# SIA-IDE/MMGT

Measured on AMD Instinct MI355X. Metric: UNet3D denoise-steps/sec at 512x512x24 bf16, higher is better.
Workload: dtype bf16; 1 GPU; BASELINE configs[1]: 512x512x24 pose2vid denoise step (CFG batch 2, UNet3D + MM-HAA, 16 reference banks, 1 window of 24 frames, guidance 3.5, DDIM v-pred), random-init weights; frames=24, parallelism=clip-parallel x1

## Files before the change

include/mmgt_hip.h:

```cpp
#ifndef MMGT_HIP_H
#define MMGT_HIP_H

#ifdef __cplusplus
extern "C" {
#endif

#define MMGT_F32 0
#define MMGT_BF16 1

#define MMGT_ACT_NONE 0
#define MMGT_ACT_GEGLU 1
#define MMGT_ACT_SILU 2
#define MMGT_ACT_RELU 3
#define MMGT_ACT_QUICK_GELU 4
#define MMGT_ACT_GELU 5
#define MMGT_ACT_MISH 6

int mmgt_abi_version(void);
const char* mmgt_last_error(void);
int mmgt_tune(const char* key, int value);
int mmgt_tune_get(const char* key, int* value);
int mmgt_box_calib(float warm_seconds, float* mfma_mhz, float* mfma_tflops, void* stream);
void mmgt_gemm16_set_trace(void* p);
void mmgt_ffn_set_trace(void* p);
// ... 84 lines not shown
                       int F, int hw, float guidance, float sa_t, float sb_t, float sa_p, float sb_p, void* stream);

int mmgt_accumulate_window(const void* pred, float* pred_sum, float* counter, const int* idx, int Fw, int F, int C,
                           int Cpad, int hw, int dtype, void* stream);

int mmgt_accumulate_window_rows(const void* pred, float* pred_sum, float* counter, const int* idx, int Fw, int F, int C,
                                int Cpad, int hw, int rows, int row0, int bump_counter, int dtype, void* stream);

int mmgt_accumulate_windows(const void* pred, float* pred_sum, float* counter, const int* idx, int B, int Fw, int F, int C, int Cpad,
                            int hw, int dtype, void* stream);

int mmgt_rotary(const void* x, const float* cos_sin, void* out, long rows, int dim, int seq, int dtype, void* stream);
int mmgt_film_residual(const void* x, const float* scale_shift, long ld_ss, const void* res, const void* res2, void* out, long rows,
                       int dim, int rows_per_batch, int dtype, void* stream);
int mmgt_mean_tokens(const void* x, float* out, int batch, int tokens, int dim, int dtype, void* stream);
int mmgt_activation(const void* x, void* out, long n, int act, int dtype, void* stream);
int mmgt_smga_ddim_step(const void* pred_uncond, const void* pred_cond, const float* x, const float* noise, float* out, long n,
                        float guidance, float sqrt_recip_acp, float sqrt_recipm1_acp, float sqrt_acp_next, float c, float sigma,
                        int last, int dtype, void* stream);

long mmgt_temporal_leg320_image_bytes(void);
int mmgt_temporal_leg320(const void* x, void* out, const float* ln_gamma, const float* beta_pe, int pe_rows, const void* wimg, const float* bias_o,
                         int batch, int frames, int n_pix, float scale, float eps, int dtype, void* stream);

long mmgt_gn_silu_conv3x3_image_bytes(int cin, int cout);
int mmgt_gn_silu_conv3x3(const void* x, const float* scale, const float* shift, const void* wimg, const float* bias, const void* residual, void* out,
                         float* stats, int nb, int H, int W, int cin, int cout, int ldo, int dtype, void* stream);
int mmgt_gn_stats_finalize(const float* stats, const float* gamma, const float* beta, float* scale, float* shift, int nb, int tiles, int C, int G,
                           float eps, void* stream);

long mmgt_gn_silu_conv3x3_unet_image_bytes(int cin, int cout);
int mmgt_gn_silu_conv3x3_unet_stats_rows(int nb, int H, int W, int cout);
int mmgt_gn_silu_conv3x3_unet_stats(const void* x0, int C0, const void* x1, int C1, const float* scale_shift, const void* wimg, const float* bias,
                                    const float* bias2, int b2_imgs, const void* residual, void* out, float* stats, int nb, int H, int W, int cout, int dtype,
                                    void* stream);
int mmgt_gn_stats_finalize_unet(const float* stats, const float* gamma, const float* beta, float* scale_shift, int nb, int parts_per_img, int count, int C,
                                int G, float eps, void* stream);
void mmgt_rconv_set_trace(void* buf);
int mmgt_gn_silu_conv3x3_unet(const void* x0, int C0, const void* x1, int C1, const float* scale_shift, const void* wimg, const float* bias,
                              const float* bias2, int b2_imgs, const void* residual, void* out, int nb, int H, int W, int cout, int dtype, void* stream);

int mmgt_blur_mask_u8(const unsigned char* masks, unsigned char* out, int frames, int H, int W, int ksize, void* stream);
int mmgt_resample_u8(const unsigned char* in, float* out_f32, unsigned char* out_u8, int frames, int S, int D, const int* bounds,
                     const int* coeffs, int ksize, void* stream);
int mmgt_window_stack(const float* x, float* out, int frames, long D, int half, void* stream);
int mmgt_frames_to_u8(const void* x, unsigned char* out, long npix, int cpad, float scale, float shift, int dtype, void* stream);
// ... 59 lines not shown
```

mmgt_amd/csrc/gemm.hip:

```cpp
#include <string.h>

#include <type_traits>

#include "common.h"
#include "gemm_common.h"
#include "mmgt_hip.h"

#ifndef MMGT_GEMM_VARIANT
#define MMGT_GEMM_VARIANT 7
#endif

namespace {

constexpr bool V_FRAGDB = (MMGT_GEMM_VARIANT & 1) != 0;
constexpr bool V_ILV = (MMGT_GEMM_VARIANT & 2) != 0;
constexpr bool V_LATE = (MMGT_GEMM_VARIANT & 4) != 0;
constexpr bool V_LATE_ALL = (MMGT_GEMM_VARIANT & 8) != 0;
constexpr bool V_NODMA = (MMGT_GEMM_VARIANT & 16) != 0;

template <int CTRL>
__device__ __forceinline__ unsigned dpp_quad(unsigned v) {
  return (unsigned)__builtin_amdgcn_mov_dpp((int)v, CTRL, 0xf, 0xf, true);
}
template <int S>
// ... 738 lines not shown
  MMGT_CHECK(M > 0 && N > 0 && K > 0, "gemm: empty problem M=%d N=%d K=%d", M, N, K);
  MMGT_CHECK(K % 64 == 0, "gemm: K=%d must be a multiple of 64 (pad channels on the host)", K);
  MMGT_CHECK(act >= 0 && act <= 6, "gemm: bad act %d", act);
  MMGT_CHECK(act != 1 || N % 64 == 0, "gemm: GEGLU needs N %% 64 == 0 (N=%d)", N);
  return 0;
}

}

void mmgt_attn_set64(int v);
void mmgt_gn_set_rows(int v);
void mmgt_attn_set_heads_inner(int v);
void mmgt_attn_set_attn80(int v);
void mmgt_attn_set_nomax(int v);
void mmgt_gemm16_set_pb(int v);
void mmgt_gemm16_set_stagger(int v);
void mmgt_gn_set_interleave(int v);
void mmgt_gn_set_lpr0(int v);
void mmgt_gn_set_narrow(int v);
void mmgt_gn_set_slab(int v);
void mmgt_ffn_set_dbg(int v);
void mmgt_rowgemm_set_dbg(int v);
void mmgt_tleg_set_abl(int v);
void mmgt_gnconv_set_abl(int v);
void mmgt_rconv_set_abl(int v);
void mmgt_rconv_set_stagger(int v);
void mmgt_rconv_set_cb(int v);
namespace {
struct HostSwitch { const char* key; int value; };
HostSwitch g_host[] = {
    {"fused_ff", 1},
    {"twin_attention", 1},
    {"shared_rows", 1},
    {"oz3", 1},
    {"rowgemm", 1},
    {"tleg", 1},
    {"rconv", 5},
    {"conv_out_taps", 1},
    {"ffpo_cat", 1},
    {"sc_cat", 1},
    {"up2", 1},
    {"rconv_stats", 1},
    {"gnconv", 2},
    {"zero_audio_skip", 1},
    {"window_state", 1},
    {"smga_graph", 1},
};
}
extern "C" int mmgt_tune_get(const char* key, int* value) {
  if (key && value)
    for (const HostSwitch& h : g_host)
      if (!strcmp(key, h.key)) { *value = h.value; return 0; }
  mmgt_set_error("tune_get: unknown key");
  return 1;
}
extern "C" int mmgt_tune(const char* key, int value) {
  if (key)
    for (HostSwitch& h : g_host)
      if (!strcmp(key, h.key)) { h.value = value; return 0; }
  if (key && !strcmp(key, "gemm_cfg")) { g_gemm_cfg = value; return 0; }
  if (key && !strcmp(key, "attn64")) { mmgt_attn_set64(value); return 0; }
  if (key && !strcmp(key, "attn_nomax") && (value == 0 || value == 1)) { mmgt_attn_set_nomax(value); return 0; }
  if (key && !strcmp(key, "attn_heads_inner")) { mmgt_attn_set_heads_inner(value); return 0; }
  if (key && !strcmp(key, "attn80")) { mmgt_attn_set_attn80(value); return 0; }
  if (key && !strcmp(key, "g16_pb")) { mmgt_gemm16_set_pb(value); return 0; }
  if (key && !strcmp(key, "g16_stagger")) { mmgt_gemm16_set_stagger(value); return 0; }
  if (key && !strcmp(key, "gn_rows")) { mmgt_gn_set_rows(value); return 0; }
  if (key && !strcmp(key, "gn_interleave")) { mmgt_gn_set_interleave(value); return 0; }
  if (key && !strcmp(key, "gn_narrow")) { mmgt_gn_set_narrow(value); return 0; }
  if (key && !strcmp(key, "gn_slab")) { mmgt_gn_set_slab(value); return 0; }
  if (key && !strcmp(key, "gn_lpr0")) { if (value != 4 && value != 8 && value != 16) return -1; mmgt_gn_set_lpr0(value); return 0; }
  if (key && !strcmp(key, "splitk")) { g_splitk = value; return 0; }
  if (key && !strcmp(key, "bm192")) { g_bm192 = value; return 0; }
  if (key && !strcmp(key, "tailsplit")) { g_tailsplit = value; return 0; }
  if (key && !strcmp(key, "rconv_cb") && (value == 0 || value == 320 || value == 256 || value == 160)) { mmgt_rconv_set_cb(value); return 0; }
  if (key && !strcmp(key, "rconv_stagger") && value >= 0 && value <= 8192) { mmgt_rconv_set_stagger(value); return 0; }
#ifdef MMGT_ABLATE
  if (key && !strcmp(key, "ffn_dbg") && value >= 0 && value <= 2) { mmgt_ffn_set_dbg(value); return 0; }
  if (key && !strcmp(key, "gnconv_abl") && value >= 0 && value <= 255) { mmgt_gnconv_set_abl(value); return 0; }
  if (key && !strcmp(key, "tleg_abl") && value >= 0 && value <= 128) { mmgt_tleg_set_abl(value); return 0; }
  if (key && !strcmp(key, "rconv_abl") && value >= 0 && value <= 31) { mmgt_rconv_set_abl(value); return 0; }
  if (key && !strcmp(key, "rowgemm_dbg") && value >= 0 && value <= 5) { mmgt_rowgemm_set_dbg(value); return 0; }
#else
  if (key && !strcmp(key, "rowgemm_dbg") && (value == 0 || value == 5)) { mmgt_rowgemm_set_dbg(value); return 0; }
  if (key && (!strcmp(key, "ffn_dbg") || !strcmp(key, "gnconv_abl") || !strcmp(key, "tleg_abl") || !strcmp(key, "rconv_abl") || !strcmp(key, "rowgemm_dbg"))) {
    mmgt_set_error("tune: '%s' selects a timing ablation whose results are garbage; the product library does not contain them (build libmmgt_hip_abl.so with `make -C mmgt_amd/csrc abl` and load it through MMGT_LIB)", key);
    return 1;
  }
#endif
// ... 156 lines not shown
```

mmgt_amd/hip.py:

```python
import ctypes
import os
from ctypes import c_float, c_int, c_long, c_void_p

import torch

_HERE = os.path.dirname(os.path.abspath(__file__))
LIB_PATH = os.environ.get("MMGT_LIB") or os.path.join(_HERE, "libmmgt_hip.so")

F32, BF16 = 0, 1
ACT_NONE, ACT_GEGLU, ACT_SILU, ACT_RELU, ACT_QUICK_GELU, ACT_GELU, ACT_MISH = 0, 1, 2, 3, 4, 5, 6

_lib = None
DMA_LIMIT = (1 << 31) - 1

_SIGS = {
    "mmgt_abi_version": (c_int, []),
    "mmgt_last_error": (ctypes.c_char_p, []),
    "mmgt_tune": (c_int, [ctypes.c_char_p, c_int]),
    "mmgt_tune_get": (c_int, [ctypes.c_char_p, ctypes.POINTER(c_int)]),
    "mmgt_box_calib": (c_int, [c_float, ctypes.POINTER(c_float), ctypes.POINTER(c_float), c_void_p]),
    "mmgt_gemm16_set_trace": (None, [c_void_p]),
    "mmgt_ffn_set_trace": (None, [c_void_p]),
    "mmgt_rconv_set_trace": (None, [c_void_p]),
    "mmgt_gemm": (c_int, [c_void_p, c_long, c_void_p, c_void_p, c_void_p, c_int, c_void_p, c_float, c_void_p, c_long,
# ... 32 lines not shown
    "mmgt_ff_fused": (c_int, [c_void_p, c_long, c_void_p, c_void_p, c_float, c_void_p, c_void_p, c_void_p, c_long, c_void_p, c_long,
                              c_int, c_int, c_int, c_int, c_void_p]),
    "mmgt_rowgemm320_image_bytes": (c_long, [c_int]),
    "mmgt_rowgemm_set_trace": (None, [c_void_p]),
    "mmgt_ff_fused_po": (c_int, [c_void_p, c_long, c_void_p, c_void_p, c_float, c_void_p, c_void_p, c_void_p, c_long, c_void_p, c_void_p,
                                 c_void_p, c_long, c_void_p, c_long, c_int, c_int, c_int, c_int, c_void_p]),
    "mmgt_groupnorm_affine": (c_int, [c_void_p, c_int, c_void_p, c_void_p, c_void_p, c_void_p, c_void_p, c_int, c_int, c_int, c_float, c_int,
                                      c_void_p]),
    "mmgt_rowgemm320": (c_int, [c_void_p, c_long, c_int, c_void_p, c_void_p, c_int, c_int, c_float, c_void_p, c_void_p, c_void_p, c_int, c_void_p,
                                c_long, c_void_p, c_long, c_int, c_void_p, c_int, c_int, c_int, c_int, c_int, c_void_p]),
    "mmgt_gn_silu_conv3x3_image_bytes": (c_long, [c_int, c_int]),
    "mmgt_gn_silu_conv3x3": (c_int, [c_void_p, c_void_p, c_void_p, c_void_p, c_void_p, c_void_p, c_void_p, c_void_p, c_int, c_int, c_int, c_int, c_int, c_int, c_int, c_void_p]),
    "mmgt_gn_silu_conv3x3_unet_image_bytes": (c_long, [c_int, c_int]),
    "mmgt_gn_silu_conv3x3_unet": (c_int, [c_void_p, c_int, c_void_p, c_int, c_void_p, c_void_p, c_void_p, c_void_p, c_int, c_void_p, c_void_p,
                                          c_int, c_int, c_int, c_int, c_int, c_void_p]),
    "mmgt_gn_silu_conv3x3_unet_stats_rows": (c_int, [c_int, c_int, c_int, c_int]),
    "mmgt_gn_silu_conv3x3_unet_stats": (c_int, [c_void_p, c_int, c_void_p, c_int, c_void_p, c_void_p, c_void_p, c_void_p, c_int, c_void_p, c_void_p, c_void_p,
                                                c_int, c_int, c_int, c_int, c_int, c_void_p]),
    "mmgt_gn_stats_finalize_unet": (c_int, [c_void_p, c_void_p, c_void_p, c_void_p, c_int, c_int, c_int, c_int, c_int, c_float, c_void_p]),
    "mmgt_groupnorm_affine2": (c_int, [c_void_p, c_int, c_void_p, c_int, c_void_p, c_void_p, c_void_p, c_void_p, c_void_p, c_int, c_int, c_int,
                                       c_float, c_int, c_void_p]),
    "mmgt_gn_stats_finalize": (c_int, [c_void_p, c_void_p, c_void_p, c_void_p, c_void_p, c_int, c_int, c_int, c_int, c_float, c_void_p]),
    "mmgt_temporal_leg320_image_bytes": (c_long, []),
    "mmgt_temporal_leg320": (c_int, [c_void_p, c_void_p, c_void_p, c_void_p, c_int, c_void_p, c_void_p, c_int, c_int, c_int, c_float, c_float, c_int,
                                     c_void_p]),
    "mmgt_channel_norm_gelu": (c_int, [c_void_p, c_void_p, c_void_p, c_void_p, c_int, c_int, c_float, c_int, c_void_p]),
    "mmgt_lerp_rows": (c_int, [c_void_p, c_void_p, c_int, c_int, c_int, c_int, c_void_p]),
    "mmgt_relpos_attention": (c_int, [c_void_p, c_long, c_long, c_void_p, c_long, c_long, c_void_p, c_long, c_long, c_void_p, c_long, c_long,
                                      c_void_p, c_long, c_long, c_void_p, c_void_p, c_void_p, c_void_p, c_int, c_int, c_int, c_int, c_float,
                                      c_int, c_void_p]),
    "mmgt_silu": (c_int, [c_void_p, c_void_p, c_long, c_int, c_void_p]),
    "mmgt_cfg_ddim_step": (c_int, [c_void_p, c_void_p, c_void_p, c_void_p, c_long, c_int, c_int, c_float, c_float,
                                   c_float, c_float, c_float, c_void_p]),
    "mmgt_accumulate_window": (c_int, [c_void_p, c_void_p, c_void_p, c_void_p, c_int, c_int, c_int, c_int, c_int, c_int,
                                       c_void_p]),
    "mmgt_rotary": (c_int, [c_void_p, c_void_p, c_void_p, c_long, c_int, c_int, c_int, c_void_p]),
    "mmgt_film_residual": (c_int, [c_void_p, c_void_p, c_long, c_void_p, c_void_p, c_void_p, c_long, c_int, c_int, c_int, c_void_p]),
    "mmgt_mean_tokens": (c_int, [c_void_p, c_void_p, c_int, c_int, c_int, c_int, c_void_p]),
    "mmgt_activation": (c_int, [c_void_p, c_void_p, c_long, c_int, c_int, c_void_p]),
    "mmgt_smga_ddim_step": (c_int, [c_void_p, c_void_p, c_void_p, c_void_p, c_void_p, c_long, c_float, c_float, c_float, c_float,
                                    c_float, c_float, c_int, c_int, c_void_p]),
    "mmgt_blur_mask_u8": (c_int, [c_void_p, c_void_p, c_int, c_int, c_int, c_int, c_void_p]),
    "mmgt_resample_u8": (c_int, [c_void_p, c_void_p, c_void_p, c_int, c_int, c_int, c_void_p, c_void_p, c_int, c_void_p]),
    "mmgt_window_stack": (c_int, [c_void_p, c_void_p, c_int, c_long, c_int, c_void_p]),
    "mmgt_frames_to_u8": (c_int, [c_void_p, c_void_p, c_long, c_int, c_float, c_float, c_int, c_void_p]),
    "mmgt_jpeg_dct_quant": (c_int, [c_void_p, c_void_p, c_int, c_int, c_int, c_int, c_int, c_void_p]),
# ... 498 lines not shown

def temporal_leg320_supported(dtype, C, heads, frames, n_pix, batch=1):
    return dtype == torch.bfloat16 and C == 320 and heads == 8 and frames in (12, 24) and n_pix % (4 * 48 // frames) == 0 and \
        batch * frames * n_pix * 640 < (1 << 31)


def temporal_leg320(x, ln_gamma, beta_pe, wimg, bias_o, batch, frames, n_pix, scale, eps=1e-5, out=None):
    _dev(x, ln_gamma, beta_pe, wimg, bias_o, out)
    if not (x.dim() == 2 and temporal_leg320_supported(x.dtype, x.shape[1], 8, frames, n_pix, batch)):
        raise RuntimeError(f"temporal_leg320: unsupported shape (dtype {x.dtype}, {tuple(x.shape)}, {frames} frames x {n_pix} pixels x batch {batch}): "
                           "8 heads of 40 channels, 12 or 24 frames, bf16, < 2 GiB")
    assert x.dim() == 2 and x.shape == (batch * frames * n_pix, 320) and x.is_contiguous() and x.dtype == torch.bfloat16
    assert wimg.dtype == torch.uint8 and wimg.is_contiguous() and wimg.numel() == lib().mmgt_temporal_leg320_image_bytes()
    assert beta_pe.dim() == 2 and beta_pe.shape[1] == 320 and beta_pe.shape[0] >= frames
    if out is None:
        out = torch.empty_like(x)
    assert out.shape == x.shape and out.is_contiguous() and out.dtype == x.dtype
    _check(lib().mmgt_temporal_leg320(_ptr(x), _ptr(out), _ptr(_f32(ln_gamma, "ln_gamma")), _ptr(_f32(beta_pe, "beta_pe")), beta_pe.shape[0],
                                      _ptr(wimg), _ptr(_f32(bias_o, "bias_o")), batch, frames, n_pix, scale, eps, dtype_code(x.dtype), _stream()),
           "mmgt_temporal_leg320")
    return out



def attention(q, k, v, out, *, batch, heads, hd, nq, nk, scale, q_str, k_str, v_str, o_str, bdiv=1, v_transposed=False,
              k2=None, v2=None, k2_str=(0, 0), v2_str=(0, 0), k2_bdiv=1, nk2=0, seg2_first_batch=0, out_scale=None, out_scale_heads=0,
              twin_out=None):
    _dev(q, k, v, out, k2, v2, out_scale, twin_out)
    if twin_out is not None:
        assert k2 is not None and v_transposed and seg2_first_batch == 0 and out_scale is None and twin_out.dtype == out.dtype
        _check(lib().mmgt_attention_twin(_ptr(q), q_str[0], q_str[1], q_str[2], _ptr(k), k_str[0], k_str[1], k_str[2], _ptr(v),
                                         v_str[0], v_str[1], v_str[2], _ptr(out), _ptr(twin_out), o_str[0], o_str[1], o_str[2], bdiv,
                                         _ptr(k2), _ptr(v2), k2_str[0], k2_str[1], v2_str[0], v2_str[1], k2_bdiv, nk2, batch, heads, hd,
                                         nq, nk, scale, dtype_code(q.dtype), _stream()), "mmgt_attention_twin")
        return out
    if out_scale is not None:
        assert k2 is None and not v_transposed and bdiv == 1 and out_scale_heads > 0 and heads % out_scale_heads == 0
        assert out_scale.dtype == torch.float32 and out_scale.dim() == 2 and out_scale.stride(1) == 1
        assert out_scale.shape == (heads // out_scale_heads, batch * nq)
        _check(lib().mmgt_attention_scaled(_ptr(q), q_str[0], q_str[1], q_str[2], _ptr(k), k_str[0], k_str[1], k_str[2], _ptr(v),
                                           v_str[0], v_str[1], v_str[2], _ptr(out), o_str[0], o_str[1], o_str[2], _ptr(out_scale),
                                           out_scale.stride(0), out_scale_heads, batch, heads, hd, nq, nk, scale, dtype_code(q.dtype),
                                           _stream()), "mmgt_attention_scaled")
        return out
    _check(lib().mmgt_attention(_ptr(q), q_str[0], q_str[1], q_str[2], _ptr(k), k_str[0], k_str[1], k_str[2], _ptr(v),
                                v_str[0], v_str[1], v_str[2], _ptr(out), o_str[0], o_str[1], o_str[2], bdiv, _ptr(k2),
# ... 836 lines not shown
```

mmgt_amd/packing.py:

```python
import torch


def pack_geglu(w, b):
    n2, k = w.shape
    n = n2 // 2
    assert n % 32 == 0
    wp = w.reshape(2, n // 32, 32, k).permute(1, 0, 2, 3).reshape(n2, k).contiguous()
    bp = None if b is None else b.reshape(2, n // 32, 32).permute(1, 0, 2).reshape(n2).contiguous()
    return wp, bp


def pack_conv3x3(w, cin_pad=None, cout_pad=None):
    cout, cin = w.shape[:2]
    cin_pad = cin_pad or cin
    cout_pad = cout_pad or cout
    out = torch.zeros((cout_pad, 3, 3, cin_pad), device=w.device, dtype=w.dtype)
    out[:cout, :, :, :cin] = w.permute(0, 2, 3, 1)
    return out.contiguous()


def pack_conv3x3_up2(w):
    cout, cin = w.shape[:2]
    wf = w if w.dtype == torch.float64 else w.float()
    groups = (((0,), (1, 2)), ((0, 1), (2,)))
# ... 117 lines not shown
        for w in bf:
            chunks.append(frags(w, wide))
            chunks.append(torch.zeros(2048, device=dev, dtype=torch.uint8))
        for w in bf:
            chunks.append(frags(w, narrow))
    ch = torch.empty((C // 32, 64, 8), device=dev, dtype=torch.long)
    jj, lqq = j[None, :], lq[:, None]
    for k in range(H):
        ch[k] = HD * k + torch.where(jj < 4, 4 * lqq + jj, 16 + 4 * lqq + jj - 4)
    for u in range(2):
        head = 4 * u + torch.where(jj < 4, 0, 2) + (lqq >= 2).long()
        ch[8 + u] = HD * head + 32 + 4 * (lqq & 1) + (jj & 3)
    wob = wo.to(torch.bfloat16)
    nt = torch.arange(2, device=dev)
    for oc in range(C // 32):
        rows = 32 * oc + 16 * nt[:, None] + lm[None, :]
        img = wob[rows[None, :, :, None], ch[:, None, :, :]]
        chunks.append(img.contiguous().view(torch.uint8).reshape(-1))
    out = torch.cat(chunks)
    assert out.numel() == 4 * (3 * 32768 + 3 * 20480) + 10 * 20480
    return out


def pack_gnconv(w):
    cout, cin = w.shape[0], w.shape[1]
    assert tuple(w.shape) == (cout, cin, 3, 3) and (cin, cout) in ((128, 128), (256, 128), (256, 256), (128, 64))
    dev = w.device
    cl = min(cout, 128)
    lane = torch.arange(64, device=dev)
    rows = 16 * torch.arange(cl // 16, device=dev)[:, None] + (lane & 15)[None, :]
    kk = torch.arange(4, device=dev)
    cols = 32 * kk[:, None, None] + 8 * (lane >> 4)[None, :, None] + torch.arange(8, device=dev)[None, None, :]
    wt = w.to(torch.bfloat16).permute(2, 3, 0, 1).reshape(9, cout, cin)
    img = torch.stack([torch.stack([wt[:, cl * blk + rows[None, :, :, None], 128 * ph + cols[:, None, :, :]] for ph in range(cin // 128)])
                       for blk in range(cout // cl)])
    return img.contiguous().view(torch.uint8).reshape(-1)


def pack_rconv(w):
    cout, cin = w.shape[0], w.shape[1]
    assert tuple(w.shape) == (cout, cin, 3, 3) and cin % 64 == 0 and cout % 16 == 0
    wt = w.to(torch.bfloat16).permute(2, 3, 0, 1).reshape(9, cout // 16, 16, cin // 64, 2, 4, 8)
    img = wt.permute(3, 0, 4, 1, 5, 2, 6)
    return img.contiguous().view(torch.uint8).reshape(-1)
```

mmgt_amd/unet3d.py:

```python
import math
from dataclasses import dataclass
from typing import Dict, List, Optional, Union

import torch

from . import hip
from .packing import pack_conv3x3, pack_conv3x3_up2, pack_conv_taps, pack_ff_fused, pack_ff_proj_out, pack_geglu, pack_rconv, pack_rowgemm, pack_tleg, pad_cols, pad_rows, round_up
from .unet3d_spec import unet3d_spec

SD15_CONFIG = dict(
    in_channels=4, out_channels=4, block_out_channels=(320, 640, 1280, 1280), layers_per_block=2, attention_head_dim=8,
    cross_attention_dim=768, audio_attention_dim=768, norm_num_groups=32, norm_eps=1e-5, center_input_sample=False,
    use_motion_module=True, use_audio_module=True, use_inflated_groupnorm=True,
    motion_module_kwargs=dict(num_attention_heads=8, temporal_position_encoding_max_len=32),
)


@dataclass
class UNet3DConditionOutput:
    sample: torch.Tensor

    def __getitem__(self, i):
        return (self.sample,)[i]


RCONV_LEVEL = {320: 1, 640: 2, 1280: 4}


class _Config(dict):
    __getattr__ = dict.__getitem__
# ... 62 lines not shown
        self.config = _Config(cfg)
        boc = tuple(cfg["block_out_channels"])
        if len(boc) != 4 or any(c % 64 for c in boc) or any((c // 8) not in (40, 80, 160) for c in boc):
            raise ValueError(f"block_out_channels {boc}: the HIP kernels cover head dims 40/80/160 (SD-1.5 widths)")
        self.boc = boc
        self.heads = 8
        self.in_channels = cfg["in_channels"]
        self.out_channels = cfg["out_channels"]
        self._device = torch.device(device)
        self._dtype = dtype
        hip.dtype_code(dtype)
        self.training = True
        self.gradient_checkpointing = False
        self._fuse_ff = bool(hip.tune_get("fused_ff"))
        self._twin = bool(hip.tune_get("twin_attention"))
        self._share_rows = bool(hip.tune_get("shared_rows"))
        self._fuse_oz = bool(hip.tune_get("oz3"))
        self._fuse_ln = bool(hip.tune_get("rowgemm"))
        self._ffpo_cat = bool(hip.tune_get("ffpo_cat"))
        self._ffpo = {}
        self._sc_cat = bool(hip.tune_get("sc_cat"))
        self._up2 = bool(hip.tune_get("up2"))
        self._fuse_tleg = bool(hip.tune_get("tleg"))
        self._rconv_stats = bool(hip.tune_get("rconv_stats"))
        self._rconv = hip.tune_get("rconv")
        self.spec = unet3d_spec(boc, cfg["cross_attention_dim"], cfg["audio_attention_dim"], self.in_channels,
                                self.out_channels, cfg["layers_per_block"],
                                cfg["motion_module_kwargs"].get("temporal_position_encoding_max_len", 32))
        self.w: Dict[str, torch.Tensor] = {}
        self._banks: Dict[str, tuple] = {}
        self.bank_fp16_roundtrip = dtype == torch.float32
        self._loaded = False
        self._ehs_cache = None
        self._zbias = {}

    @classmethod
    def from_config(cls, config, **kwargs):
        config = dict(config)
        config.update(kwargs)
        dev = config.pop("device", "cuda")
        dt = config.pop("dtype", torch.bfloat16)
        return cls(device=dev, dtype=dt, **config)

    @classmethod
    def from_pretrained_2d(cls, pretrained_model_path, motion_module_path, subfolder=None, unet_additional_kwargs=None,
                           mm_zero_proj_out=False, device="cuda", dtype=torch.bfloat16):
# ... 236 lines not shown
                w[t + ".oz3.wb"] = self._t(pad).contiguous()
            ff(t + ".ff")

        self._motion = [k[: -len(".temporal_transformer.norm.weight")] for k in self.spec
                        if k.endswith(".temporal_transformer.norm.weight")]
        for p in self._motion:
            q = p + ".temporal_transformer"
            t = q + ".transformer_blocks.0"
            norm(q + ".norm")
            lin(q + ".proj_in")
            proj_in_img(q)
            lin(q + ".proj_out")
            for i in range(2):
                a = f"{t}.attention_blocks.{i}"
                if has(a + ".to_q.weight"):
                    w[a + ".qkv.w"] = self._t(torch.cat([sd[a + ".to_q.weight"], sd[a + ".to_k.weight"],
                                                         sd[a + ".to_v.weight"]], 0))
                    rowimg(a + ".qkv_img", [sd[a + ".to_q.weight"], sd[a + ".to_k.weight"], sd[a + ".to_v.weight"]])
                    if self._fuse_tleg and has(a + ".to_out.0.weight") and has(a + ".to_out.0.bias") and \
                            hip.temporal_leg320_supported(self._dtype, sd[a + ".to_q.weight"].shape[1], self.heads, 24, 4096):
                        w[a + ".tleg_img"] = pack_tleg(*(sd[a + k].to(self._device) for k in (".to_q.weight", ".to_k.weight", ".to_v.weight",
                                                                                               ".to_out.0.weight")))
                lin(a + ".to_out.0", a + ".o")
                if has(a + ".pos_encoder.pe"):
                    w[a + ".pe"] = self._f(sd[a + ".pos_encoder.pe"][0])
                norm(f"{t}.norms.{i}")
                if (a + ".pe") in w and (f"{t}.norms.{i}.b") in w:
                    w[f"{t}.norms.{i}.bpe"] = (w[f"{t}.norms.{i}.b"][None, :] + w[a + ".pe"]).contiguous()
            norm(t + ".ff_norm")
            ff(t + ".ff")

    def bank_keys(self) -> List[str]:
        down = [p for p in self._spatial if p.startswith("down_blocks")]
        up = [p for p in self._spatial if p.startswith("up_blocks")]
        mid = [p for p in self._spatial if p.startswith("mid_block")]
        return down + up + mid

    def set_banks(self, banks: Optional[Dict[str, torch.Tensor]]):
        self._banks = {}
        if not banks:
            return
        for p, bank in banks.items():
            if p not in self._spatial:
                raise KeyError(f"set_banks: {p} is not a reference-attention reader")
            t = p + ".transformer_blocks.0.attn1"
            bk = bank.to(self._device)
# ... 340 lines not shown
    def _motion_module(self, p, x, frames):
        nb, h, ww, c = x.shape
        n = h * ww
        m = nb * n
        b = nb // frames
        hd = c // self.heads
        if frames > 32:
            raise RuntimeError("temporal attention window is limited to 32 frames (positional encoding max_len)")
        q = p + ".temporal_transformer"
        t = q + ".transformer_blocks.0"
        hid = self._norm_proj_in(q, x)
        for i in range(2):
            a = f"{t}.attention_blocks.{i}"
            if (a + ".tleg_img") in self.w and (f"{t}.norms.{i}.bpe") in self.w and hip.temporal_leg320_supported(self._dtype, c, self.heads, frames, n, b):
                hid = hip.temporal_leg320(hid, self.w[f"{t}.norms.{i}.g"], self.w[f"{t}.norms.{i}.bpe"], self.w[a + ".tleg_img"], self.w[a + ".o.bias"],
                                          b, frames, n, hd ** -0.5)
                continue
            if (a + ".qkv_img") in self.w and n % 128 == 0:
                qkv, _ = hip.rowgemm320(hid, self.w[a + ".qkv_img"], 3 * c, ln_gamma=self.w[f"{t}.norms.{i}.g"],
                                        ln_beta=self.w[f"{t}.norms.{i}.bpe"], pe_div=n, pe_mod=frames)
            else:
                nrm = hip.layernorm(hid, self.w[f"{t}.norms.{i}.g"], self.w[f"{t}.norms.{i}.bpe"], 1e-5, pe_div=n, pe_mod=frames)
                qkv = hip.gemm(nrm, self.w[a + ".qkv.w"])
            o = torch.empty((m, c), device=self._device, dtype=self._dtype)
            st = (frames * n * 3 * c, 3 * c, n * 3 * c)
            hip.attention(qkv, qkv[:, c:], qkv[:, 2 * c:], o, batch=b * n, heads=self.heads, hd=hd, nq=frames, nk=frames,
                          scale=hd ** -0.5, q_str=st, k_str=st, v_str=st, o_str=(frames * n * c, c, n * c), bdiv=n)
            hid = hip.gemm(o, self.w[a + ".o.w"], self.w[a + ".o.bias"], residual=hid)
        out = self._norm_ff_proj_out(t + ".ff", t + ".ff_norm", hid, q, x.view(m, c))
        return out.view(nb, h, ww, c)

    def _time_embedding(self, timestep, batch):
        if not torch.is_tensor(timestep):
            ts = torch.tensor([float(timestep)], dtype=torch.float32, device=self._device)
        else:
            ts = timestep.to(device=self._device, dtype=torch.float32).reshape(-1)
        if ts.numel() == 1:
            batch = 1
        ts = ts.expand(batch).contiguous()
        feat = hip.timestep_features(ts, self.boc[0], self._dtype)
        e = self._lin("time_embedding.linear_1", feat, act=hip.ACT_SILU)
        e = self._lin("time_embedding.linear_2", e)
        all_t = hip.gemm(hip.silu(e), self.w["temb_all.w"], self.w["temb_all.bias"]).float()
        return {p: all_t[:, off:off + n].contiguous() for p, (off, n) in self._temb_slices.items()}

    def forward(self, sample, timestep, encoder_hidden_states, audio_embedding=None, class_labels=None,
# ... 110 lines not shown
```

Before: 15.04 steps/s.

## Fuse temporal attention, output projection, bias and residual into one kernel

Adds a HIP kernel for temporal self-attention at the 640- and 1280-channel levels. Each block does the per-pixel 24-frame attention for all 8 heads into LDS, then runs the output-projection GEMM from a prepacked weight image, adding bias and the residual. This drops the attention-output round trip to global memory and one GEMM launch per temporal leg. The default switch value enables it only for the 640-channel level; it also adds an optional sleep-based stagger for the first wave of blocks and extra weight memory for the packed images.

```diff
diff --git a/include/mmgt_hip.h b/include/mmgt_hip.h
--- a/include/mmgt_hip.h
+++ b/include/mmgt_hip.h
@@ -130,6 +130,10 @@
 long mmgt_temporal_leg320_image_bytes(void);
 int mmgt_temporal_leg320(const void* x, void* out, const float* ln_gamma, const float* beta_pe, int pe_rows, const void* wimg, const float* bias_o,
                          int batch, int frames, int n_pix, float scale, float eps, int dtype, void* stream);
+
+long mmgt_temporal_tail_image_bytes(int C);
+int mmgt_temporal_tail(const void* qkv, const void* hid, void* out, const void* wimg, const float* bias_o, int batch, int frames, int n_pix,
+                       int C, int heads, float scale, int dtype, void* stream);
 
 long mmgt_gn_silu_conv3x3_image_bytes(int cin, int cout);
 int mmgt_gn_silu_conv3x3(const void* x, const float* scale, const float* shift, const void* wimg, const float* bias, const void* residual, void* out,
diff --git a/mmgt_amd/csrc/gemm.hip b/mmgt_amd/csrc/gemm.hip
--- a/mmgt_amd/csrc/gemm.hip
+++ b/mmgt_amd/csrc/gemm.hip
@@ -784,6 +784,7 @@
 void mmgt_ffn_set_dbg(int v);
 void mmgt_rowgemm_set_dbg(int v);
 void mmgt_tleg_set_abl(int v);
+void mmgt_ttail_set_stagger(int v);
 void mmgt_gnconv_set_abl(int v);
 void mmgt_rconv_set_abl(int v);
 void mmgt_rconv_set_stagger(int v);
@@ -797,6 +798,7 @@
     {"oz3", 1},
     {"rowgemm", 1},
     {"tleg", 1},
+    {"ttail", 1},
     {"rconv", 5},
     {"conv_out_taps", 1},
     {"ffpo_cat", 1},
@@ -827,6 +829,7 @@
   if (key && !strcmp(key, "attn80")) { mmgt_attn_set_attn80(value); return 0; }
   if (key && !strcmp(key, "g16_pb")) { mmgt_gemm16_set_pb(value); return 0; }
   if (key && !strcmp(key, "g16_stagger")) { mmgt_gemm16_set_stagger(value); return 0; }
+  if (key && !strcmp(key, "ttail_stagger") && value >= -1 && value <= 16) { mmgt_ttail_set_stagger(value); return 0; }
   if (key && !strcmp(key, "gn_rows")) { mmgt_gn_set_rows(value); return 0; }
   if (key && !strcmp(key, "gn_interleave")) { mmgt_gn_set_interleave(value); return 0; }
   if (key && !strcmp(key, "gn_narrow")) { mmgt_gn_set_narrow(value); return 0; }
diff --git a/mmgt_amd/csrc/ttail.hip b/mmgt_amd/csrc/ttail.hip
--- /dev/null
+++ b/mmgt_amd/csrc/ttail.hip
@@ -0,0 +1,332 @@
+#include <type_traits>
+
+#include "common.h"
+#include "gemm_common.h"
+#include "mmgt_hip.h"
+
+namespace {
+
+typedef __attribute__((ext_vector_type(4))) float acc4;
+
+constexpr int TT_HEADS = 8, TT_GT = 10, TT_RING = 16;
+
+struct TtailArgs {
+  const bf16_t* qkv;
+  const bf16_t* hid;
+  bf16_t* out;
+  const char* wimg;
+  const float* bias;
+  int n, tasks_per_batch;
+  unsigned qkv_bytes, hid_bytes, img_bytes;
+  float scale_log2e;
+  int stagger, first_round;
+};
+
+__device__ __forceinline__ acc4 tt_mma(s16x8 a, s16x8 b, acc4 c) { return __builtin_amdgcn_mfma_f32_16x16x32_bf16(a, b, c, 0, 0, 0); }
+__device__ __forceinline__ s16x8 tt_frag(u32x4 u) {
+  union { u32x4 u; s16x8 s; } cv;
+  cv.u = u;
+  return cv.s;
+}
+__device__ __forceinline__ s16x8 tt_frag2(u32x2 lo, u32x2 hi) { return tt_frag((u32x4){lo[0], lo[1], hi[0], hi[1]}); }
+__device__ __forceinline__ u32x2 tt_pack4(acc4 v) { return (u32x2){pack_bf16x2(v[0], v[1]), pack_bf16x2(v[2], v[3])}; }
+__device__ __forceinline__ float tt_lo(unsigned u) { return __uint_as_float(u << 16); }
+__device__ __forceinline__ float tt_hi(unsigned u) { return __uint_as_float(u & 0xffff0000u); }
+__device__ __forceinline__ float tt_quad_sum(float v) {
+  const auto a = __builtin_amdgcn_permlane16_swap(__float_as_uint(v), __float_as_uint(v), false, false);
+  v = __uint_as_float(a[0]) + __uint_as_float(a[1]);
+  const auto b = __builtin_amdgcn_permlane32_swap(__float_as_uint(v), __float_as_uint(v), false, false);
+  return __uint_as_float(b[0]) + __uint_as_float(b[1]);
+}
+__device__ __forceinline__ float tt_quad_max(float v) {
+  const auto a = __builtin_amdgcn_permlane16_swap(__float_as_uint(v), __float_as_uint(v), false, false);
+  v = fmaxf(__uint_as_float(a[0]), __uint_as_float(a[1]));
+  const auto b = __builtin_amdgcn_permlane32_swap(__float_as_uint(v), __float_as_uint(v), false, false);
+  return fmaxf(__uint_as_float(b[0]), __uint_as_float(b[1]));
+}
+
+template <int F> constexpr bool tt_pair(int kt, int qt) { return (16 * kt) / F <= (16 * qt + 15) / F && (16 * qt) / F <= (16 * kt + 15) / F; }
+template <int F> constexpr bool tt_all(int kt, int qt) { return (16 * kt) / F == (16 * kt + 15) / F && (16 * qt) / F == (16 * qt + 15) / F && (16 * kt) / F == (16 * qt) / F; }
+
+template <int C> constexpr int tt_rows() { return C == 640 ? 48 : 24; }
+template <int C> constexpr int tt_lds() { return tt_rows<C>() * (C * 2 + 16); }
+
+template <int C, int F>
+__global__ __launch_bounds__(256) __attribute__((amdgpu_waves_per_eu(2, 2)))
+void ttail_kernel(const TtailArgs a) {
+  constexpr int R = tt_rows<C>(), NRT = (R + 15) / 16, P = R / F;
+  constexpr int HD = C / TT_HEADS, KSH = (HD + 31) / 32, NCH = HD / 16;
+  constexpr int RS = C * 2 + 16, NKS = C / 32, NG = C / (4 * 16 * TT_GT);
+  static_assert(R % F == 0 && F % 4 == 0 && HD % 16 == 0 && NKS % 2 == 0 && NG >= 1, "geometry");
+  extern __shared__ __attribute__((aligned(16))) char smem[];
+  const int tid = threadIdx.x, lane = tid & 63, wid = __builtin_amdgcn_readfirstlane(tid >> 6);
+  const int lm = lane & 15, lq = lane >> 4;
+  using std::integral_constant;
+#define TT_IC(v) integral_constant<int, (v)>{}
+  auto for_range = [](auto LOc, auto HIc, auto&& fn) {
+    constexpr int lo = decltype(LOc)::value, hi = decltype(HIc)::value;
+    [&]<int... I>(std::integer_sequence<int, I...>) { (fn(integral_constant<int, lo + I>{}), ...); }(std::make_integer_sequence<int, (hi > lo ? hi - lo : 0)>{});
+  };
+
+  const __amdgpu_buffer_rsrc_t rq = __builtin_amdgcn_make_buffer_rsrc(const_cast<bf16_t*>(a.qkv), 0, (int)a.qkv_bytes, 0x00020000);
+  const __amdgpu_buffer_rsrc_t rh = __builtin_amdgcn_make_buffer_rsrc(const_cast<bf16_t*>(a.hid), 0, (int)a.hid_bytes, 0x00020000);
+  const __amdgpu_buffer_rsrc_t ro = __builtin_amdgcn_make_buffer_rsrc(a.out, 0, (int)a.hid_bytes, 0x00020000);
+  const __amdgpu_buffer_rsrc_t rw = __builtin_amdgcn_make_buffer_rsrc(const_cast<char*>(a.wimg), 0, (int)a.img_bytes, 0x00020000);
+
+  if (a.stagger > 0 && (int)blockIdx.x >= a.first_round / 2 && (int)blockIdx.x < a.first_round) {
+    for (int i = 0; i < a.stagger; ++i) __builtin_amdgcn_s_sleep(127);
+  }
+
+  const int task = blockIdx.x;
+  const int b = task / a.tasks_per_batch, p0 = (task - b * a.tasks_per_batch) * P;
+  unsigned qoff[NRT], hoff[NRT];
+#pragma unroll
+  for (int rt = 0; rt < NRT; ++rt) {
+    const int rho = 16 * rt + lm, rc = rho < R ? rho : R - 1;
+    const int px = rc / F, f = rc - px * F;
+    const unsigned grow = (unsigned)((b * F + f) * a.n + p0 + px);
+    qoff[rt] = grow * (unsigned)(3 * C * 2);
+    hoff[rt] = grow * (unsigned)(C * 2);
+  }
+  unsigned tmask = 0;
+#pragma unroll
+  for (int qt = 0; qt < NRT; ++qt)
+#pragma unroll
+    for (int kt = 0; kt < NRT; ++kt)
+      if ((16 * kt + 4 * lq) / F == (16 * qt + lm) / F) tmask |= 1u << (NRT * qt + kt);
+  s16x8 sel[2];
+#pragma unroll
+  for (int half = 0; half < 2; ++half)
+#pragma unroll
+    for (int j = 0; j < 8; ++j) sel[half][j] = (8 * lq + j == lm + 16 * half) ? (short)0x3F80 : (short)0;
+
+  const int cofs = 16 * (lq & 1) + 8 * (lq >> 1);
+  auto load_res = [&](auto& rv, auto GTc, int tile0) {
+    constexpr int GT = decltype(GTc)::value;
+#pragma unroll
+    for (int c2 = 0; c2 < GT / 2; ++c2)
+#pragma unroll
+      for (int rt = 0; rt < NRT; ++rt) rv[c2][rt] = __builtin_amdgcn_raw_buffer_load_b128(rh, (int)(hoff[rt] + (unsigned)(((tile0 + 2 * c2) * 16 + cofs) * 2)), 0, 0);
+  };
+  auto load_piece = [&](s16x8 (&dst)[NRT][KSH], int piece, int h) {
+#pragma unroll
+    for (int rt = 0; rt < NRT; ++rt)
+#pragma unroll
+      for (int ks = 0; ks < KSH; ++ks) {
+        const bool whole = 32 * ks + 32 <= HD;
+        const bool ok = whole || 32 * ks + 8 * lq < HD;
+        const int ch = h * HD + 32 * ks + 8 * (ok ? lq : 0);
+        u32x4 v = __builtin_amdgcn_raw_buffer_load_b128(rq, (int)(qoff[rt] + (unsigned)((piece * C + ch) * 2)), 0, 0);
+        if (!ok) v = (u32x4)(0u);
+        dst[rt][ks] = tt_frag(v);
+      }
+  };
+  auto transpose_v = [&](u32x2 (&vp)[NRT][NCH], const s16x8 (&vf)[NRT][KSH]) {
+#pragma unroll
+    for (int rt = 0; rt < NRT; ++rt)
+#pragma unroll
+      for (int ct = 0; ct < NCH; ++ct) vp[rt][ct] = tt_pack4(tt_mma(vf[rt][ct / 2], sel[ct & 1], (acc4)(0.f)));
+  };
+  const u32x2 z2 = (u32x2){0u, 0u};
+  auto attend = [&](int h, const s16x8 (&qf)[NRT][KSH], const s16x8 (&kf)[NRT][KSH], const u32x2 (&vp)[NRT][NCH]) {
+    for_range(TT_IC(0), TT_IC(NRT), [&](auto qc) {
+      constexpr int qt = decltype(qc)::value;
+      acc4 s[NRT];
+      float mx = -1e30f;
+      for_range(TT_IC(0), TT_IC(NRT), [&](auto kc) {
+        constexpr int kt = decltype(kc)::value;
+        if constexpr (tt_pair<F>(kt, qt)) {
+          acc4 t = (acc4)(0.f);
+#pragma unroll
+          for (int ks = 0; ks < KSH; ++ks) t = tt_mma(kf[kt][ks], qf[qt][ks], t);
+          if constexpr (!tt_all<F>(kt, qt)) {
+            const bool ok = (tmask >> (NRT * qt + kt)) & 1u;
+#pragma unroll
+            for (int e = 0; e < 4; ++e) t[e] = ok ? t[e] : -1e30f;
+          }
+#pragma unroll
+          for (int e = 0; e < 4; ++e) mx = fmaxf(mx, t[e]);
+          s[kt] = t;
+        }
+      });
+      mx = tt_quad_max(mx);
+      const float nm = -mx * a.scale_log2e;
+      float ls = 0.f;
+      u32x2 pp[3] = {z2, z2, z2};
+      for_range(TT_IC(0), TT_IC(NRT), [&](auto kc) {
+        constexpr int kt = decltype(kc)::value;
+        if constexpr (tt_pair<F>(kt, qt)) {
+          acc4 e4;
+#pragma unroll
+          for (int e = 0; e < 4; ++e) {
+            e4[e] = __builtin_amdgcn_exp2f(fmaf(s[kt][e], a.scale_log2e, nm));
+            ls += e4[e];
+          }
+          pp[kt] = tt_pack4(e4);
+        }
+      });
+      const float inv = 1.f / tt_quad_sum(ls);
+      const int rho = 16 * qt + lm;
+      char* orow = smem + rho * RS + (h * HD + 4 * lq) * 2;
+#pragma unroll
+      for (int ct = 0; ct < NCH; ++ct) {
+        acc4 o = tt_mma(tt_frag2(vp[0][ct], vp[1][ct]), tt_frag2(pp[0], pp[1]), (acc4)(0.f));
+        if constexpr (NRT == 3) {
+          if constexpr (tt_pair<F>(2, qt)) o = tt_mma(tt_frag2(vp[NRT - 1][ct], z2), tt_frag2(pp[2], z2), o);
+        }
+        if (rho < R) *reinterpret_cast<u32x2*>(orow + ct * 32) = tt_pack4(o * inv);
+      }
+    });
+  };
+  constexpr int GT0 = NRT == 3 ? 6 : TT_GT, GT1 = NRT == 3 ? 4 : TT_GT;
+  u32x4 rv0[GT0 / 2][NRT], rv1[GT1 / 2][NRT];
+  {
+    const int hA = 2 * wid, hB = hA + 1;
+    s16x8 qa[NRT][KSH], ka[NRT][KSH], va[NRT][KSH];
+    u32x2 vpa[NRT][NCH];
+    load_piece(va, 2, hA);
+    load_piece(ka, 1, hA);
+    load_piece(qa, 0, hA);
+    __builtin_amdgcn_sched_barrier(0);
+    transpose_v(vpa, va);
+    __builtin_amdgcn_sched_barrier(0);
+    s16x8 qb[NRT][KSH], kb[NRT][KSH], vb[NRT][KSH];
+    u32x2 vpb[NRT][NCH];
+    load_piece(vb, 2, hB);
+    load_piece(kb, 1, hB);
+    __builtin_amdgcn_sched_barrier(0);
+    attend(hA, qa, ka, vpa);
+    __builtin_amdgcn_sched_barrier(0);
+    load_piece(qb, 0, hB);
+    load_res(rv0, TT_IC(GT0), wid * NG * TT_GT);
+    if constexpr (NRT == 3) load_res(rv1, TT_IC(GT1), wid * TT_GT + GT0);
+    __builtin_amdgcn_sched_barrier(0);
+    transpose_v(vpb, vb);
+    attend(hB, qb, kb, vpb);
+  }
+  __syncthreads();
+
+  int brow[NRT];
+#pragma unroll
+  for (int rt = 0; rt < NRT; ++rt) brow[rt] = ((16 * rt + lm) < R ? 16 * rt + lm : R - 1) * RS + 16 * lq;
+  auto out_group = [&](auto GTc, int G, int c0, const auto& rv) {
+    constexpr int GT = decltype(GTc)::value;
+    static_assert(GT % 2 == 0, "tiles are stored in pairs");
+    const int tile0 = G * TT_GT + c0;
+    acc4 acc[GT][NRT];
+#pragma unroll
+    for (int c = 0; c < GT; ++c) {
+      const acc4 bv = *reinterpret_cast<const acc4*>(a.bias + (tile0 + c) * 16 + 4 * lq);
+#pragma unroll
+      for (int rt = 0; rt < NRT; ++rt) acc[c][rt] = bv;
+    }
+    const int wbase = (G * NKS * TT_GT + c0) * 1024 + lane * 16;
+    s16x8 ring[TT_RING];
+#pragma unroll
+    for (int i = 0; i < TT_RING; ++i) ring[i] = tt_frag(__builtin_amdgcn_raw_buffer_load_b128(rw, wbase + ((i / GT) * TT_GT + i % GT) * 1024, 0, 0));
+    s16x8 bf[2][NRT];
+#pragma unroll
+    for (int rt = 0; rt < NRT; ++rt) bf[0][rt] = *reinterpret_cast<const s16x8*>(smem + brow[rt]);
+    for_range(TT_IC(0), TT_IC(NKS), [&](auto kc) {
+      constexpr int ks = decltype(kc)::value;
+      if constexpr (ks + 1 < NKS) {
+#pragma unroll
+        for (int rt = 0; rt < NRT; ++rt) bf[(ks + 1) & 1][rt] = *reinterpret_cast<const s16x8*>(smem + brow[rt] + (ks + 1) * 64);
+      }
+      for_range(TT_IC(0), GTc, [&](auto cc) {
+        constexpr int c = decltype(cc)::value, i = ks * GT + c, nx = i + TT_RING;
+#pragma unroll
+        for (int rt = 0; rt < NRT; ++rt) acc[c][rt] = tt_mma(ring[i % TT_RING], bf[ks & 1][rt], acc[c][rt]);
+        if constexpr (nx < NKS * GT)
+          ring[i % TT_RING] = tt_frag(__builtin_amdgcn_raw_buffer_load_b128(rw, wbase + ((nx / GT) * TT_GT + nx % GT) * 1024, 0, 0));
+        __builtin_amdgcn_sched_barrier(0);
+      });
+    });
+#pragma unroll
+    for (int c2 = 0; c2 < GT / 2; ++c2) {
+      const unsigned col2 = (unsigned)(((tile0 + 2 * c2) * 16 + cofs) * 2);
+#pragma unroll
+      for (int rt = 0; rt < NRT; ++rt) {
+        if (16 * rt + lm < R) {
+          float o8[8];
+#pragma unroll
+          for (int r = 0; r < 4; ++r) {
+            const auto sw = __builtin_amdgcn_permlane16_swap(__float_as_uint(acc[2 * c2][rt][r]), __float_as_uint(acc[2 * c2 + 1][rt][r]), false, false);
+            o8[r] = __uint_as_float(sw[0]);
+            o8[4 + r] = __uint_as_float(sw[1]);
+          }
+#pragma unroll
+          for (int j = 0; j < 4; ++j) {
+            o8[2 * j] += tt_lo(rv[c2][rt][j]);
+            o8[2 * j + 1] += tt_hi(rv[c2][rt][j]);
+          }
+          const u32x4 pk = (u32x4){pack_bf16x2(o8[0], o8[1]), pack_bf16x2(o8[2], o8[3]), pack_bf16x2(o8[4], o8[5]), pack_bf16x2(o8[6], o8[7])};
+          __builtin_amdgcn_raw_buffer_store_b128(pk, ro, (int)(hoff[rt] + col2), 0, MMGT_ST_AUX);
+        }
+      }
+    }
+  };
+  if constexpr (NRT == 3) {
+    out_group(TT_IC(GT0), wid, 0, rv0);
+    out_group(TT_IC(GT1), wid, GT0, rv1);
+  } else {
+    static_assert(NRT == 3 || NG == 2, "1280 channels: two ten-tile groups per wave");
+    out_group(TT_IC(TT_GT), wid * NG, 0, rv0);
+    load_res(rv1, TT_IC(GT1), (wid * NG + 1) * TT_GT);
+    out_group(TT_IC(TT_GT), wid * NG + 1, 0, rv1);
+  }
+#undef TT_IC
+}
+
+int g_ttail_stagger = -1;
+
+}
+
+void mmgt_ttail_set_stagger(int v) { g_ttail_stagger = v; }
+
+extern "C" long mmgt_temporal_tail_image_bytes(int C) { return (C == 640 || C == 1280) ? (long)C * C * 2 : 0; }
+
+extern "C" int mmgt_temporal_tail(const void* qkv, const void* hid, void* out, const void* wimg, const float* bias_o, int batch, int frames,
+                                  int n_pix, int C, int heads, float scale, int dtype, void* stream) {
+  MMGT_CHECK(qkv && hid && out && wimg && bias_o, "temporal_tail: null pointer");
+  MMGT_CHECK(dtype == MMGT_BF16, "temporal_tail: bf16 only (the fp32-I/O mode runs mmgt_attention -> GEMM + residual)");
+  MMGT_CHECK((C == 640 || C == 1280) && heads == TT_HEADS, "temporal_tail: built for 8 heads over 640 or 1280 channels, got %d heads over %d (level 0 is mmgt_temporal_leg320)", heads, C);
+  MMGT_CHECK(frames == 24 || frames == 12, "temporal_tail: built for windows of 24 or 12 frames, got %d", frames);
+  const int P = (C == 640 ? 48 : 24) / frames;
+  MMGT_CHECK(batch > 0 && n_pix > 0 && n_pix % P == 0, "temporal_tail: pixels per frame (%d) must be a multiple of %d", n_pix, P);
+  MMGT_CHECK((long)batch * frames * n_pix * 3 * C * 2 < (1l << 31), "temporal_tail: tensor beyond the 2 GiB range of a buffer resource (split the batch)");
+  MMGT_CHECK((((uintptr_t)qkv | (uintptr_t)hid | (uintptr_t)out | (uintptr_t)wimg | (uintptr_t)bias_o) & 15) == 0, "temporal_tail: pointers must be 16-byte aligned");
+  const long rows = (long)batch * frames * n_pix;
+  {
+    const char *q0 = (const char*)qkv, *q1 = q0 + rows * 3 * C * 2, *o0 = (const char*)out, *o1 = o0 + rows * C * 2;
+    MMGT_CHECK(o1 <= q0 || q1 <= o0, "temporal_tail: out overlaps q | k | v (other tasks still read them)");
+    MMGT_CHECK(out == hid || (const char*)hid + rows * C * 2 <= o0 || o1 <= (const char*)hid, "temporal_tail: out may alias the residual only exactly");
+  }
+  TtailArgs a;
+  a.qkv = (const bf16_t*)qkv; a.hid = (const bf16_t*)hid; a.out = (bf16_t*)out; a.wimg = (const char*)wimg; a.bias = bias_o;
+  a.n = n_pix; a.tasks_per_batch = n_pix / P;
+  a.qkv_bytes = (unsigned)(rows * 3 * C * 2); a.hid_bytes = (unsigned)(rows * C * 2); a.img_bytes = (unsigned)((long)C * C * 2);
+  a.scale_log2e = scale * 1.4426950408889634f;
+  const unsigned grid = (unsigned)(batch * a.tasks_per_batch);
+  int dev = 0;
+  static int ncu[16] = {};
+  MMGT_CHECK(hipGetDevice(&dev) == hipSuccess && dev >= 0 && dev < 16, "temporal_tail: device query failed");
+  if (!ncu[dev]) {
+    hipDeviceProp_t prop;
+    MMGT_CHECK(hipGetDeviceProperties(&prop, dev) == hipSuccess, "temporal_tail: device query failed");
+    ncu[dev] = prop.multiProcessorCount;
+  }
+  a.first_round = 2 * ncu[dev];
+  a.stagger = g_ttail_stagger >= 0 ? g_ttail_stagger : (int)grid <= ncu[dev] ? 0 : (int)((double)rows * C * 8 / 2 / 4.3e6 / 3.4 + 0.5);
+  if (a.stagger > 16) a.stagger = 16;
+  hipStream_t s = (hipStream_t)stream;
+  if (C == 640) {
+    if (frames == 24) hipLaunchKernelGGL((ttail_kernel<640, 24>), dim3(grid), dim3(256), (size_t)tt_lds<640>(), s, a);
+    else hipLaunchKernelGGL((ttail_kernel<640, 12>), dim3(grid), dim3(256), (size_t)tt_lds<640>(), s, a);
+  } else {
+    if (frames == 24) hipLaunchKernelGGL((ttail_kernel<1280, 24>), dim3(grid), dim3(256), (size_t)tt_lds<1280>(), s, a);
+    else hipLaunchKernelGGL((ttail_kernel<1280, 12>), dim3(grid), dim3(256), (size_t)tt_lds<1280>(), s, a);
+  }
+  MMGT_LAUNCH_CHECK();
+  return 0;
+}
diff --git a/mmgt_amd/hip.py b/mmgt_amd/hip.py
--- a/mmgt_amd/hip.py
+++ b/mmgt_amd/hip.py
@@ -78,6 +78,8 @@
                                        c_float, c_int, c_void_p]),
     "mmgt_gn_stats_finalize": (c_int, [c_void_p, c_void_p, c_void_p, c_void_p, c_void_p, c_int, c_int, c_int, c_int, c_float, c_void_p]),
     "mmgt_temporal_leg320_image_bytes": (c_long, []),
+    "mmgt_temporal_tail_image_bytes": (c_long, [c_int]),
+    "mmgt_temporal_tail": (c_int, [c_void_p, c_void_p, c_void_p, c_void_p, c_void_p, c_int, c_int, c_int, c_int, c_int, c_float, c_int, c_void_p]),
     "mmgt_temporal_leg320": (c_int, [c_void_p, c_void_p, c_void_p, c_void_p, c_int, c_void_p, c_void_p, c_int, c_int, c_int, c_float, c_float, c_int,
                                      c_void_p]),
     "mmgt_channel_norm_gelu": (c_int, [c_void_p, c_void_p, c_void_p, c_void_p, c_int, c_int, c_float, c_int, c_void_p]),
@@ -622,6 +624,29 @@
     return out
 
 
+def temporal_tail_supported(dtype, C, heads, frames, n_pix, batch=1):
+    return dtype == torch.bfloat16 and C in (640, 1280) and heads == 8 and frames in (12, 24) and n_pix > 0 and batch > 0 and \
+        n_pix % ((48 if C == 640 else 24) // frames) == 0 and batch * frames * n_pix * 6 * C < (1 << 31)
+
+
+def temporal_tail(qkv, hid, wimg, bias_o, batch, frames, n_pix, heads, scale, out=None):
+    _dev(qkv, hid, wimg, bias_o, out)
+    C = hid.shape[1] if hid.dim() == 2 else 0
+    if not temporal_tail_supported(hid.dtype, C, heads, frames, n_pix, batch):
+        raise RuntimeError(f"temporal_tail: unsupported shape (dtype {hid.dtype}, {tuple(hid.shape)}, {heads} heads, {frames} frames x {n_pix} pixels x "
+                           f"batch {batch}): 8 heads over 640 or 1280 channels, 12 or 24 frames, whole tasks, bf16, < 2 GiB")
+    M = batch * frames * n_pix
+    assert qkv.shape == (M, 3 * C) and qkv.is_contiguous() and qkv.dtype == hid.dtype
+    assert hid.shape == (M, C) and hid.is_contiguous()
+    assert wimg.dtype == torch.uint8 and wimg.is_contiguous() and wimg.numel() == lib().mmgt_temporal_tail_image_bytes(C)
+    if out is None:
+        out = torch.empty_like(hid)
+    assert out.shape == hid.shape and out.is_contiguous() and out.dtype == hid.dtype
+    _check(lib().mmgt_temporal_tail(_ptr(qkv), _ptr(hid), _ptr(out), _ptr(wimg), _ptr(_f32(bias_o, "bias_o")), batch, frames, n_pix, C, heads,
+                                    scale, dtype_code(hid.dtype), _stream()), "mmgt_temporal_tail")
+    return out
+
+
 
 def attention(q, k, v, out, *, batch, heads, hd, nq, nk, scale, q_str, k_str, v_str, o_str, bdiv=1, v_transposed=False,
               k2=None, v2=None, k2_str=(0, 0), v2_str=(0, 0), k2_bdiv=1, nk2=0, seg2_first_batch=0, out_scale=None, out_scale_heads=0,
diff --git a/mmgt_amd/packing.py b/mmgt_amd/packing.py
--- a/mmgt_amd/packing.py
+++ b/mmgt_amd/packing.py
@@ -163,6 +163,13 @@
     return out
 
 
+def pack_ttail(w_o):
+    C = w_o.shape[0]
+    assert tuple(w_o.shape) == (C, C) and C in (640, 1280)
+    img = w_o.to(torch.bfloat16).reshape(C // 160, 10, 16, C // 32, 4, 8).permute(0, 3, 1, 4, 2, 5).contiguous()
+    return img.view(torch.uint8).reshape(-1)
+
+
 def pack_gnconv(w):
     cout, cin = w.shape[0], w.shape[1]
     assert tuple(w.shape) == (cout, cin, 3, 3) and (cin, cout) in ((128, 128), (256, 128), (256, 256), (128, 64))
diff --git a/mmgt_amd/unet3d.py b/mmgt_amd/unet3d.py
--- a/mmgt_amd/unet3d.py
+++ b/mmgt_amd/unet3d.py
@@ -5,7 +5,7 @@
 import torch
 
 from . import hip
-from .packing import pack_conv3x3, pack_conv3x3_up2, pack_conv_taps, pack_ff_fused, pack_ff_proj_out, pack_geglu, pack_rconv, pack_rowgemm, pack_tleg, pad_cols, pad_rows, round_up
+from .packing import pack_conv3x3, pack_conv3x3_up2, pack_conv_taps, pack_ff_fused, pack_ff_proj_out, pack_geglu, pack_rconv, pack_rowgemm, pack_tleg, pack_ttail, pad_cols, pad_rows, round_up
 from .unet3d_spec import unet3d_spec
 
 SD15_CONFIG = dict(
@@ -114,6 +114,7 @@
         self._sc_cat = bool(hip.tune_get("sc_cat"))
         self._up2 = bool(hip.tune_get("up2"))
         self._fuse_tleg = bool(hip.tune_get("tleg"))
+        self._ttail = int(hip.tune_get("ttail"))
         self._rconv_stats = bool(hip.tune_get("rconv_stats"))
         self._rconv = hip.tune_get("rconv")
         self.spec = unet3d_spec(boc, cfg["cross_attention_dim"], cfg["audio_attention_dim"], self.in_channels,
@@ -396,6 +397,9 @@
                         w[a + ".tleg_img"] = pack_tleg(*(sd[a + k].to(self._device) for k in (".to_q.weight", ".to_k.weight", ".to_v.weight",
                                                                                                ".to_out.0.weight")))
                 lin(a + ".to_out.0", a + ".o")
+                if self._ttail and self._dtype == torch.bfloat16 and has(a + ".to_out.0.weight") and has(a + ".to_out.0.bias") and \
+                        sd[a + ".to_out.0.weight"].shape[0] in (640, 1280):
+                    w[a + ".ttail_img"] = pack_ttail(sd[a + ".to_out.0.weight"].to(self._device))
                 if has(a + ".pos_encoder.pe"):
                     w[a + ".pe"] = self._f(sd[a + ".pos_encoder.pe"][0])
                 norm(f"{t}.norms.{i}")
@@ -782,6 +786,10 @@
             else:
                 nrm = hip.layernorm(hid, self.w[f"{t}.norms.{i}.g"], self.w[f"{t}.norms.{i}.bpe"], 1e-5, pe_div=n, pe_mod=frames)
                 qkv = hip.gemm(nrm, self.w[a + ".qkv.w"])
+            if (a + ".ttail_img") in self.w and self._ttail & (1 if c == 640 else 2 if n > 64 else 4) and \
+                    hip.temporal_tail_supported(self._dtype, c, self.heads, frames, n, b):
+                hid = hip.temporal_tail(qkv, hid, self.w[a + ".ttail_img"], self.w[a + ".o.bias"], b, frames, n, self.heads, hd ** -0.5)
+                continue
             o = torch.empty((m, c), device=self._device, dtype=self._dtype)
             st = (frames * n * 3 * c, 3 * c, n * 3 * c)
             hip.attention(qkv, qkv[:, c:], qkv[:, 2 * c:], o, batch=b * n, heads=self.heads, hd=hd, nq=frames, nk=frames,
```

Result: no change. 15.04 steps/s (median of 2 runs) (-0.0%).
